# ljishen/bitar

Hardware: AMD Instinct MI355X
Metric: GiB/s compress+decompress on 1-GiB Arrow buffer, 1/2/4/8 GPUs; % HBM roofline (higher is better)
Workload: dtype u8; 1 GPU; LZ4 block compress + decompress round trip, 1 GiB per GPU, 64 KiB segments, Silesia-style mix (BASELINE configs[2]); bytes_per_gpu=1073741824, segment_bytes=65536, segments_per_gpu=16384, codec=lz4-block, input_kind=1, parallelism=1 GPU

## Files before the change

### bitar_amd/csrc/compress.hip

```cpp
#include "window_parse.hip.h"

namespace bitar_hip {

namespace cmp {

__device__ __forceinline__ uint32_t lane_sel(uint64_t m, uint32_t a, uint32_t b) {
  uint32_t r;
  __asm__("v_cndmask_b32_e64 %0, %1, %2, %3" : "=v"(r) : "v"(b), "v"(a), "s"(m));
  return r;
}

#ifndef BITAR_LZ4_GATHER
#define BITAR_LZ4_GATHER 2
#endif
#ifndef BITAR_LZ4_OBUF
#define BITAR_LZ4_OBUF 512
#endif
constexpr uint32_t kLz4Obuf = BITAR_LZ4_OBUF;
constexpr uint32_t kSeqCap = 64;
struct Lz4Lds {
#if BITAR_LZ4_GATHER == 2
  uint8_t ring[kLz4Obuf];
#else
  uint8_t ring[kLz4Obuf + kWave];
#endif
  uint2 seqs[kSeqCap + 1];
  uint32_t marks[kWave + 1];
};

struct Lz4Out : ByteOutT<kLz4Obuf> {
  Lz4Lds* L;
  uint32_t nseq;
  uint32_t last_end;
  uint32_t step_id;

  __device__ __forceinline__ void init(Lz4Lds* lds, GMEM uint8_t* d, uint64_t c) {
    L = lds;
    ring = lds->ring;
    dst = d;
    cap = c;
    op = flushed = 0;
    overflow = false;
    nseq = 0;
    last_end = 0;
    step_id = 0;
    lds->marks[lane_id()] = 0;
    lds_order();
  }
  __device__ __forceinline__ void put_ext(uint32_t v) {
    const uint32_t cnt = v / 255u + 1;
    for (uint32_t k = 0; k < cnt; k += kWave) {
      const uint32_t step = cnt - k < kWave ? cnt - k : kWave;
      if (!room(step)) return;
      const uint32_t t = k + lane_id();
      put(t + 1 < cnt ? 255u : v % 255u, step);
    }
  }
  __device__ __forceinline__ void one(const GMEM uint8_t* in, const InRing& I, uint32_t lit_start,
                                      uint32_t lit_len, uint32_t off, uint32_t mlen) {
    if (overflow) return;
    const uint32_t ml = mlen ? mlen - kMinMatch : 0;
    const uint32_t token = ((lit_len < 15 ? lit_len : 15) << 4) | (ml < 15 ? ml : 15);
    if (!room(1)) return;
    put(token, 1);
    if (lit_len >= 15) put_ext(lit_len - 15);
    if (overflow) return;
    if (lit_len) {
      if ((uint64_t)op + lit_len > cap) { overflow = true; return; }
      if (lit_len <= 256 && lit_start >= I.lo) {
        for (uint32_t k = 0; k < lit_len; k += kWave) {
          const uint32_t step = lit_len - k < kWave ? lit_len - k : kWave;
          room(step);
          lds_order();
          const uint32_t b = I.byte(lit_start + k + (lane_id() < step ? lane_id() : 0u));
          put(b, step);
        }
      } else {
        flush(op, true);
        wave_copy_global(dst + op, in + lit_start, lit_len);
        op += lit_len;
        flushed = op;
      }
    }
    if (!mlen) return;
    if (!room(2)) return;
    put(lane_id() ? off >> 8 : off & 0xFF, 2);
    if (ml >= 15) put_ext(ml - 15);
  }

#if BITAR_LZ4_GATHER == 2
  __device__ __forceinline__ bool bulk(const InRing& I, uint32_t lo, uint32_t hi, uint32_t q,
                                       uint32_t lit_start, uint32_t off, uint32_t mlen) {
    const uint32_t lane = lane_id();
    const bool in = (lane >= lo) & (lane < hi);
    const uint32_t lit_len = q - lit_start, ml = mlen - kMinMatch;
    const uint32_t nlx = lit_len >= 15 ? 1u : 0u, nmx = ml >= 15 ? 1u : 0u;
    const uint32_t e = in ? 3u + nlx + nmx + lit_len : 0u;
    const uint32_t incl = wave_incl_sum(e);
    const uint32_t total = readlane(incl, kWave - 1);
    if ((uint64_t)op + total > cap) return false;
    const uint32_t a = incl - e;
    const uint32_t tok = ((lit_len < 15 ? lit_len : 15) << 4) | (ml < 15 ? ml : 15);
    const uint32_t A = a + nlx;
    const uint32_t T1 = a + 2u + nlx + lit_len;
    const uint32_t hb = nlx ? tok | (((lit_len - 15u) & 0xFFu) << 8) : tok << 8;
    const uint32_t D = I.in_lo + lit_start - A - 2u;
    const uint32_t pA = A | (T1 << 16);
    const uint32_t pH = hb | (D << 16);
    const uint32_t pT = (off & 0xFFFFu) | (((ml - 15u) & 0xFFu) << 16);
    const uint32_t a4 = in ? a << 2 : 0x7FFFFF00u;
    const uint32_t mark = a + 1u;
    const uint32_t zero = 0;
    const uint32_t rbase = (uint32_t)(uintptr_t)dst + op - 1u;
    uint32_t u = lane + 1u;
    uint32_t before = lo - 1u;
    for (uint32_t R = 0; R < total; R += kWave) {
      if (op + kWave - flushed > kLz4Obuf - 64) flush(op, false);
      lds_order();
      const uint32_t slot = min(a4 - (R << 2), (uint32_t)kWave << 2);
      *reinterpret_cast<uint32_t*>(reinterpret_cast<uint8_t*>(L->marks) + slot) = mark;
      lds_order();
      const uint32_t mk = L->marks[lane];
      L->marks[lane] = zero;
      const uint64_t S = ballot(mk == u);
      const uint32_t base = before + (uint32_t)(S & 1u);
      const uint64_t S1 = S >> 1;
      const uint32_t idx = __builtin_amdgcn_mbcnt_hi((uint32_t)(S1 >> 32),
                                                     __builtin_amdgcn_mbcnt_lo((uint32_t)S1, 0u));
      before += (uint32_t)__builtin_popcountll(S);
      const int src = (int)((idx << 2) + (base << 2));
      const uint32_t qA = (uint32_t)__builtin_amdgcn_ds_bpermute(src, (int)pA);
      const uint32_t qH = (uint32_t)__builtin_amdgcn_ds_bpermute(src, (int)pH);
      const uint32_t qT = (uint32_t)__builtin_amdgcn_ds_bpermute(src, (int)pT);
      const uint32_t r = u - (qA & 0xFFFFu);
      const uint32_t t = u - (qA >> 16);
      const uint32_t sel = min(min(t, r + 4u), 6u);
      const uint32_t litb = I.ring[(((u << 16) + qH) >> 16) & I.mask];
      const uint32_t hi4 = __builtin_amdgcn_perm(litb, qH, 0x0C040100u);
      const uint32_t b = __builtin_amdgcn_perm(hi4, qT, sel);
      const uint32_t nb = total - R < kWave ? total - R : kWave;
      ring[(rbase + u) & kMask] = (uint8_t)b;
      lds_order();
      op += nb;
      u += kWave;
    }
    return true;
  }
#else
  __device__ __forceinline__ bool bulk(const InRing& I, uint32_t lo, uint32_t hi, uint32_t q,
                                       uint32_t lit_start, uint32_t off, uint32_t mlen) {
    const uint32_t lane = lane_id();
    const bool in = (lane >= lo) & (lane < hi);
    const uint32_t lit_len = q - lit_start, ml = mlen - kMinMatch;
    const uint32_t nlx = lit_len >= 15 ? 1u : 0u, nmx = ml >= 15 ? 1u : 0u;
    const uint32_t e = in ? 3u + nlx + nmx + lit_len : 0u;
    const uint32_t incl = wave_incl_sum(e);
    const uint32_t total = readlane(incl, kWave - 1);
    if ((uint64_t)op + total > cap) return false;
    const uint32_t a = incl - e;
    const uint32_t tok = ((lit_len < 15 ? lit_len : 15) << 4) | (ml < 15 ? ml : 15);
    const uint32_t p0 = a | (lit_len << 16) | (nlx << 25) | (nmx << 26);
    const uint32_t p1 = lit_start | (tok << 16);
    const uint32_t p2 = (off & 0xFFFFu) | (((ml - 15u) & 0xFFu) << 16) | ((lit_len - 15u) << 24);
    for (uint32_t R = 0; R < total; R += kWave) {
      room(kWave);
      step_id += 1;
      const bool st = in & (a - R < kWave);
      lds_order();
      L->marks[st ? a - R : kWave] = (step_id << 8) | (lane + 1);
      lds_order();
      const uint32_t mk = L->marks[lane];
      const uint32_t before = (uint32_t)__builtin_popcountll(ballot(in & (a < R)));
      const uint32_t carry = before ? lo + before : 0u;
      const uint32_t v = (mk >> 8) == step_id ? (mk & 0xFFu) : 0u;
      const uint32_t s1 = max(wave_incl_max(v), carry);
      const int src = (int)((s1 - 1) << 2);
      const uint32_t q0 = (uint32_t)__builtin_amdgcn_ds_bpermute(src, (int)p0);
      const uint32_t q1 = (uint32_t)__builtin_amdgcn_ds_bpermute(src, (int)p1);
      const uint32_t q2 = (uint32_t)__builtin_amdgcn_ds_bpermute(src, (int)p2);
      const uint32_t r = R + lane - (q0 & 0xFFFFu);
      const uint32_t ll = (q0 >> 16) & 511u;
      const uint32_t L0 = 1u + ((q0 >> 25) & 1u), h = L0 + ll;
      const uint32_t litb = I.byte((q1 & 0xFFFFu) + r - L0);
      uint32_t b = r == h + 2 ? (q2 >> 16) & 0xFFu : (q2 >> 8) & 0xFFu;
      b = r == h ? q2 & 0xFFu : b;
      b = r < h ? litb : b;
      b = r < L0 ? q2 >> 24 : b;
      b = r == 0 ? (q1 >> 16) & 0xFFu : b;
      const uint32_t nb = total - R < kWave ? total - R : kWave;
      lds_order();
      ring[lane < nb ? at(op + lane) : kLz4Obuf + lane] = (uint8_t)b;
      lds_order();
      op += nb;
    }
    return true;
  }
#endif

  __device__ __forceinline__ void flush_seqs(const GMEM uint8_t* in, const InRing& I) {
    const uint32_t cnt = nseq;
    nseq = 0;
    if (!cnt || overflow) return;
    const uint32_t lane = lane_id();
    lds_order();
    const uint2 rec = L->seqs[lane < cnt ? lane : kSeqCap];
    const uint32_t q = rec.x & 0xFFFFu, off = (rec.x >> 16) + 1u, mlen = rec.y;
    const uint32_t end = q + mlen;
    const uint32_t prev = wave_shr1(end);
    const uint32_t lit_start = lane == 0 ? last_end : prev;
    const uint32_t lit_len = q - lit_start;
    last_end = readlane(end, cnt - 1);
    const uint64_t live = cnt < kWave ? (1ull << cnt) - 1 : ~0ull;
    uint64_t special = (ballot(lit_len >= 270u) | ballot(mlen >= 270u + kMinMatch) |
                        ballot(lit_start < I.lo)) & live;
    uint32_t lo = 0;
    for (;;) {
      const uint32_t k = special ? (uint32_t)__builtin_ctzll(special) : cnt;
      if (k > lo && !bulk(I, lo, k, q, lit_start, off, mlen)) {
        for (uint32_t j = lo; j < k && !overflow; ++j)
          one(in, I, readlane(lit_start, j), readlane(lit_len, j), readlane(off, j),
              readlane(mlen, j));
      }
      if (k >= cnt || overflow) break;
      one(in, I, readlane(lit_start, k), readlane(lit_len, k), readlane(off, k),
          readlane(mlen, k));
      special &= special - 1;
      lo = k + 1;
    }
  }

  __device__ __forceinline__ void sequence(const GMEM uint8_t* in, const InRing& I,
                                           uint32_t lit_start, uint32_t lit_len, uint32_t off,
                                           uint32_t mlen) {
    flush_seqs(in, I);
    one(in, I, lit_start, lit_len, off, mlen);
  }
  __device__ __forceinline__ uint32_t pending_from(uint32_t anchor, uint32_t) const { return anchor; }

  __device__ __forceinline__ void between(const GMEM uint8_t* in, const InRing& I) {
    if (nseq > kSeqCap - 16) flush_seqs(in, I);
  }
  __device__ __forceinline__ void window(const GMEM uint8_t*, const InRing&, const Window& W,
                                         uint32_t, uint32_t) {
    if (!W.chain) return;
    const uint64_t chain = W.chain;
    const uint32_t idx = __builtin_amdgcn_mbcnt_hi((uint32_t)(chain >> 32),
                                                   __builtin_amdgcn_mbcnt_lo((uint32_t)chain, nseq));
    const uint32_t lane = lane_id();
    lds_order();
    L->seqs[lane_sel(chain, idx, kSeqCap)] =
        make_uint2((W.x + lane) | (W.dm1 << 16), W.mlen);
    lds_order();
    nseq += (uint32_t)__builtin_popcountll(chain);
  }
};

constexpr uint32_t kBitWords = BITAR_CMP_BITWORDS, kBitMask = kBitWords - 1;

__device__ __forceinline__ uint32_t rev(uint32_t v, uint32_t n) {
  return __builtin_bitreverse32(v) >> (32 - n);
}
__device__ __forceinline__ uint32_t fixed_code(uint32_t s, uint32_t& n) {
  const uint32_t code = s < 144 ? 0x30 + s : s < 256 ? 0x190 + (s - 144) : s < 280 ? s - 256 : 0xC0 + (s - 280);
  n = s < 144 ? 8u : s < 256 ? 9u : s < 280 ? 7u : 8u;
  return __builtin_bitreverse32(code) >> (32 - n);
}
__device__ __forceinline__ uint32_t match_code(uint32_t mlen, uint32_t off, uint32_t& n) {
  const uint32_t v = mlen - 3;
  const uint32_t lev = 29u - __builtin_clz(v | 8u);
  const uint32_t le = mlen == 258 || v < 8 ? 0u : lev;
  const uint32_t lc = mlen == 258 ? 28u : v < 8 ? v : 4 * lev + 4 + ((v >> lev) & 3u);
  const uint32_t lx = v & ((1u << le) - 1);
  const uint32_t d = off - 1;
  const uint32_t dev = 30u - __builtin_clz(d | 4u);
  const uint32_t de = d < 4 ? 0u : dev;
  const uint32_t dc = d < 4 ? d : 2 * dev + 2 + ((d >> dev) & 1u);
  const uint32_t dx = d & ((1u << de) - 1);
  uint32_t ln;
  const uint32_t code = fixed_code(257 + lc, ln);
  n = ln + le + 5 + de;
  return code | (lx << ln) | (rev(dc, 5) << (ln + le)) | (dx << (ln + le + 5));
}

#ifndef BITAR_DFL_BULK
#define BITAR_DFL_BULK 1
#endif
struct DflLds {
  uint2 recs[kSeqCap + 1];
  uint32_t marks[kWave + 1];
};
struct DflOut {
  uint32_t* stage;
  GMEM uint32_t* dst;
  uint64_t cap;
  uint64_t bits;
  uint32_t wflushed;
  bool overflow;

  __device__ __forceinline__ void flush_words(uint32_t upto) {
    const uint32_t lane = lane_id();
    lds_order();
    for (uint32_t w = wflushed + lane; w < upto; w += kWave) {
      dst[w] = stage[w & kBitMask];
      stage[w & kBitMask] = 0;
    }
    lds_order();
    wflushed = upto;
  }
  __device__ __forceinline__ void drain() {
    const uint32_t full = (uint32_t)(bits >> 5);
    if (full != wflushed) flush_words(full);
  }
  __device__ __forceinline__ void put_lanes(uint32_t val, uint32_t nb) {
    if (overflow) return;
    const uint32_t incl = wave_incl_sum(nb);
    const uint32_t total = readlane(incl, 63);
    if ((bits + total + 7) / 8 > cap) { overflow = true; return; }
    const uint64_t bp = bits + incl - nb;
    const uint32_t w = (uint32_t)(bp >> 5), sh = (uint32_t)(bp & 31);
    const uint32_t spill = sh + nb > 32 ? val >> ((32 - sh) & 31) : 0u;
    lds_order();
    if (nb) atomicOr(&stage[w & kBitMask], val << sh);
    if (sh + nb > 32) atomicOr(&stage[(w + 1) & kBitMask], spill);
    lds_order();
    bits += total;
    const uint32_t full = (uint32_t)(bits >> 5);
    if (full - wflushed >= kBitWords - 80) flush_words(full);
  }
  __device__ __forceinline__ void put_one(uint32_t val, uint32_t nb) {
    put_lanes(lane_id() == 0 ? val : 0u, lane_id() == 0 ? nb : 0u);
  }
  __device__ __forceinline__ void literals(const GMEM uint8_t* in, const InRing& I, uint32_t s,
                                           uint32_t n) {
    const uint32_t lane = lane_id();
    const bool ring_ok = s >= I.lo;
    for (uint32_t k = 0; k < n; k += kWave) {
      const uint32_t step = n - k < kWave ? n - k : kWave;
      const uint32_t q = s + k + (lane < step ? lane : 0);
      uint32_t b;
      lds_order();
      if (ring_ok) b = I.byte(q);
      else b = lane < step ? (uint32_t)in[q] : 0u;
      uint32_t nb;
      const uint32_t code = fixed_code(b, nb);
      put_lanes(lane < step ? code : 0u, lane < step ? nb : 0u);
      if (overflow) return;
    }
  }
#if BITAR_DFL_BULK
  DflLds* L;
  uint32_t npend, last_end;

  __device__ __forceinline__ void bulk(const InRing& I, uint32_t lo, uint32_t hi,
                                       uint32_t lit_start, uint32_t ll, uint32_t mv, uint32_t mb) {
    const uint32_t lane = lane_id();
    const bool in = (lane >= lo) & (lane < hi);
    const uint32_t e = in ? ll + 1u : 0u;
    const uint32_t incl = wave_incl_sum(e);
    const uint32_t total = readlane(incl, kWave - 1);
    const uint32_t a = incl - e;
    const uint32_t D = I.in_lo + lit_start - a - 1u;
    const uint32_t pX = ((a + ll + 1u) << 16) | mb;
    const uint32_t a4 = in ? a << 2 : 0x7FFFFF00u;
    const uint32_t mark = a + 1u;
    const uint32_t zero = 0;
    uint32_t u = lane + 1u;
    uint32_t before = lo - 1u;
    for (uint32_t R = 0; R < total && !overflow; R += kWave) {
      lds_order();
      const uint32_t slot = min(a4 - (R << 2), (uint32_t)kWave << 2);
      *reinterpret_cast<uint32_t*>(reinterpret_cast<uint8_t*>(L->marks) + slot) = mark;
      lds_order();
      const uint32_t mk = L->marks[lane];
      L->marks[lane] = zero;
      const uint64_t S = ballot(mk == u);
      const uint32_t base = before + (uint32_t)(S & 1u);
      const uint64_t S1 = S >> 1;
      const uint32_t k = __builtin_amdgcn_mbcnt_hi((uint32_t)(S1 >> 32),
                                                   __builtin_amdgcn_mbcnt_lo((uint32_t)S1, 0u));
      before += (uint32_t)__builtin_popcountll(S);
      const int src = (int)((k << 2) + (base << 2));
      const uint32_t qD = (uint32_t)__builtin_amdgcn_ds_bpermute(src, (int)D);
      const uint32_t qX = (uint32_t)__builtin_amdgcn_ds_bpermute(src, (int)pX);
      const uint32_t qM = (uint32_t)__builtin_amdgcn_ds_bpermute(src, (int)mv);
      const uint32_t b = I.ring[(qD + u) & I.mask];
      uint32_t lb;
      const uint32_t lv = fixed_code(b, lb);
      const bool ism = u == (qX >> 16);
      const bool live = u <= total;
      put_lanes(ism ? qM : lv, live ? (ism ? (qX & 63u) : lb) : 0u);
      u += kWave;
    }
  }
  __device__ __forceinline__ void flush_seqs(const GMEM uint8_t* in, const InRing& I) {
    const uint32_t cnt = npend;
    npend = 0;
    if (!cnt || overflow) return;
    const uint32_t lane = lane_id();
    lds_order();
    const uint2 rec = L->recs[lane < cnt ? lane : kSeqCap];
    const uint32_t q = rec.x & 0xFFFFu, off = (rec.x >> 16) + 1u, mlen = rec.y;
    const uint32_t end = q + mlen;
    const uint32_t prev = wave_shr1(end);
    const uint32_t lit_start = lane == 0 ? last_end : prev;
    const uint32_t ll = q - lit_start;
    last_end = readlane(end, cnt - 1);
    uint32_t mb;
    const uint32_t mv = match_code(lane < cnt ? mlen : 3u, lane < cnt ? off : 1u, mb);
    const uint64_t live = cnt < kWave ? (1ull << cnt) - 1 : ~0ull;
    uint64_t special = ballot(lit_start < I.lo) & ballot(ll != 0u) & live;
    uint32_t lo = 0;
    for (;;) {
      const uint32_t k = special ? (uint32_t)__builtin_ctzll(special) : cnt;
      if (k > lo) bulk(I, lo, k, lit_start, ll, mv, mb);
      if (k >= cnt || overflow) break;
      literals(in, I, readlane(lit_start, k), readlane(ll, k));
      put_one(readlane(mv, k), readlane(mb, k));
      special &= special - 1;
      lo = k + 1;
    }
  }
  __device__ __forceinline__ uint32_t pending_from(uint32_t anchor, uint32_t) const { return anchor; }
  __device__ __forceinline__ void between(const GMEM uint8_t* in, const InRing& I) {
    if (npend > kSeqCap - 16) flush_seqs(in, I);
  }
  __device__ __forceinline__ void sequence(const GMEM uint8_t* in, const InRing& I, uint32_t s,
                                           uint32_t n, uint32_t, uint32_t) {
    flush_seqs(in, I);
    literals(in, I, s, n);
  }
  __device__ __forceinline__ void window(const GMEM uint8_t*, const InRing&, const Window& W,
                                         uint32_t, uint32_t) {
    if (!W.chain) return;
    const uint64_t chain = W.chain;
    const uint32_t idx = __builtin_amdgcn_mbcnt_hi((uint32_t)(chain >> 32),
                                                   __builtin_amdgcn_mbcnt_lo((uint32_t)chain, npend));
    const uint32_t lane = lane_id();
    lds_order();
    L->recs[lane_sel(chain, idx, kSeqCap)] =
        make_uint2((W.x + lane) | (W.dm1 << 16), W.mlen);
    lds_order();
    npend += (uint32_t)__builtin_popcountll(chain);
  }
#else
  __device__ __forceinline__ uint32_t pending_from(uint32_t, uint32_t emitted) const { return emitted; }
  __device__ __forceinline__ void between(const GMEM uint8_t*, const InRing&) {}
  __device__ __forceinline__ void sequence(const GMEM uint8_t* in, const InRing& I, uint32_t s,
                                           uint32_t n, uint32_t, uint32_t) {
    literals(in, I, s, n);
  }

  __device__ __forceinline__ void window(const GMEM uint8_t*, const InRing&, const Window& W,
                                         uint32_t, uint32_t n) {
    const uint32_t lane = lane_id();
    const uint32_t q = W.x + lane;
    const bool cl = (W.chain >> lane) & 1;
    const uint32_t pend = wave_incl_max(cl ? q + W.mlen : 0u);
    const bool covered = q < W.pos_in || (!cl && q < pend);
    uint32_t mb, lb;
    const uint32_t mv = match_code(cl ? W.mlen : 3u, cl ? W.off() : 1u, mb);
    const uint32_t lv = fixed_code(W.byte, lb);
    const bool lit = !cl && !covered && q < n;
    put_lanes(cl ? mv : lit ? lv : 0u, cl ? mb : lit ? lb : 0u);
  }
#endif
};

}

#ifndef BITAR_LZ4C_WAVES
#define BITAR_LZ4C_WAVES 0
#endif
#if BITAR_LZ4C_WAVES
#define BITAR_LZ4C_ATTR __attribute__((amdgpu_waves_per_eu(BITAR_LZ4C_WAVES)))
#else
#define BITAR_LZ4C_ATTR
#endif
template <uint32_t RING, uint32_t HLOG>
__global__ __launch_bounds__(64) BITAR_LZ4C_ATTR void lz4_compress_kernel(
    const uint8_t* __restrict__ input, uint64_t n_total, uint32_t seg,
    uint8_t* __restrict__ slab, uint64_t slot_stride, uint8_t* const* __restrict__ dsts,
    uint32_t* __restrict__ sizes, uint32_t* __restrict__ err, const uint32_t* __restrict__ order) {
  using namespace cmp;
  __shared__ __attribute__((aligned(16))) uint16_t table[(1u << HLOG) + 8];
  __shared__ __attribute__((aligned(16))) uint8_t inring[RING + kInPad];
  __shared__ __attribute__((aligned(16))) Lz4Lds olds;
  const uint32_t i_seg = order ? order[blockIdx.x] : blockIdx.x;
  const uint64_t seg_off = (uint64_t)i_seg * seg;
  if (seg_off >= n_total) return;
  const uint32_t n = (uint32_t)((n_total - seg_off) < seg ? (n_total - seg_off) : seg);
  Lz4Out o;
  o.init(&olds, global_ptr(dsts ? dsts[i_seg] : slab + (uint64_t)i_seg * slot_stride), slot_stride);
#ifndef BITAR_CMP_LZ4_SKIP
#define BITAR_CMP_LZ4_SKIP 1
#endif
  parse<Lz4Out, false, BITAR_CMP_LZ4_SKIP != 0, RING, HLOG>(global_ptr(input + seg_off), n,
                                         global_ptr(input + n_total), table, inring,
                                         RING - 1536u, 0xFFFFFFFFu, o);
  o.flush(o.op, true);
  if (lane_id() == 0) {
    sizes[i_seg] = o.overflow ? 0xFFFFFFFFu : o.op;
    if (o.overflow) atomicOr(err, 2u);
  }
}

template __global__ void lz4_compress_kernel<cmp::kIn, cmp::kHashLog>(
    const uint8_t*, uint64_t, uint32_t, uint8_t*, uint64_t, uint8_t* const*, uint32_t*, uint32_t*,
    const uint32_t*);
template __global__ void lz4_compress_kernel<16384, 12>(
    const uint8_t*, uint64_t, uint32_t, uint8_t*, uint64_t, uint8_t* const*, uint32_t*, uint32_t*,
    const uint32_t*);

template <bool BITS>
__device__ __forceinline__ void deflate_compress_body(
    const uint8_t* __restrict__ input, uint64_t n_total, uint32_t seg,
    uint8_t* __restrict__ slab, uint64_t slot_stride, uint8_t* const* __restrict__ dsts,
    uint32_t* __restrict__ sizes, uint32_t* __restrict__ err, const uint32_t* __restrict__ order,
    uint32_t* __restrict__ bits) {
  using namespace cmp;
  __shared__ __attribute__((aligned(16))) uint16_t table[1u << kHashLog];
  __shared__ __attribute__((aligned(16))) uint8_t inring[kIn + kInPad];
  __shared__ __attribute__((aligned(16))) uint32_t stage[kBitWords];
#if BITAR_DFL_BULK
  __shared__ __attribute__((aligned(16))) DflLds dl;
#endif
  const uint32_t i_seg = order ? order[blockIdx.x] : blockIdx.x;
  const uint64_t seg_off = (uint64_t)i_seg * seg;
  if (seg_off >= n_total) return;
  const uint32_t n = (uint32_t)((n_total - seg_off) < seg ? (n_total - seg_off) : seg);
  for (uint32_t k = lane_id(); k < kBitWords; k += kWave) stage[k] = 0;
  DflOut o;
  o.stage = stage;
  o.dst = reinterpret_cast<GMEM uint32_t*>(
      global_ptr(dsts ? dsts[i_seg] : slab + (uint64_t)i_seg * slot_stride));
  o.cap = slot_stride;
  o.bits = 0;
  o.wflushed = 0;
  o.overflow = false;
#if BITAR_DFL_BULK
  o.L = &dl;
  o.npend = 0;
  o.last_end = 0;
  dl.marks[lane_id()] = 0;
  lds_order();
#endif
  o.put_one(1u | (1u << 1), 3);
  parse(global_ptr(input + seg_off), n, global_ptr(input + n_total), table, inring, kMaxDist,
        258u, o);
  uint32_t eb;
  const uint32_t eob = fixed_code(256, eb);
  o.put_one(eob, eb);
  o.flush_words((uint32_t)((o.bits + 31) >> 5));
  uint32_t size = (uint32_t)((o.bits + 7) >> 3);
  uint32_t nbits = (uint32_t)o.bits;
  const uint32_t nblk = (n + 65534u) / 65535u;
  const uint32_t stored = nblk * 5u + n;
  if (!o.overflow && stored < size + (n >> 4)) {
    GMEM uint8_t* d = reinterpret_cast<GMEM uint8_t*>(o.dst);
    const GMEM uint8_t* in = global_ptr(input + seg_off);
    global_fence_wave();
    uint32_t p = 0, q = 0;
    for (uint32_t b = 0; b < nblk; ++b) {
      const uint32_t len = n - p < 65535u ? n - p : 65535u;
      const uint32_t lane = lane_id();
      const uint32_t hv = lane == 0 ? (b + 1 == nblk ? 1u : 0u)
                          : lane == 1 ? len & 0xFFu : lane == 2 ? len >> 8
                          : lane == 3 ? ~len & 0xFFu : (~len >> 8) & 0xFFu;
      if (lane < 5) d[q + lane] = (uint8_t)hv;
      wave_copy_global(d + q + 5, in + p, len);
      p += len;
      q += 5 + len;
    }
    size = stored;
    nbits = stored * 8u;
  }
  if (lane_id() == 0) {
    sizes[i_seg] = o.overflow ? 0xFFFFFFFFu : size;
    if (BITS && bits) bits[i_seg] = o.overflow ? 0xFFFFFFFFu : nbits;
    if (o.overflow) atomicOr(err, 2u);
  }
}

__global__ __launch_bounds__(64) void deflate_compress_kernel(
    const uint8_t* __restrict__ input, uint64_t n_total, uint32_t seg,
    uint8_t* __restrict__ slab, uint64_t slot_stride, uint8_t* const* __restrict__ dsts,
    uint32_t* __restrict__ sizes, uint32_t* __restrict__ err, const uint32_t* __restrict__ order) {
  deflate_compress_body<false>(input, n_total, seg, slab, slot_stride, dsts, sizes, err, order,
                               nullptr);
}

__global__ __launch_bounds__(64) void deflate_compress_bits_kernel(
    const uint8_t* __restrict__ input, uint64_t n_total, uint32_t seg,
    uint8_t* __restrict__ slab, uint64_t slot_stride, uint8_t* const* __restrict__ dsts,
    uint32_t* __restrict__ sizes, uint32_t* __restrict__ err, const uint32_t* __restrict__ order,
    uint32_t* __restrict__ bits) {
  deflate_compress_body<true>(input, n_total, seg, slab, slot_stride, dsts, sizes, err, order,
                              bits);
}

}
```

Before: 244.1 GiB/s.

## Add ring-direct LZ4 sequence emitter with mark-based literal gather

Adds a third bulk emitter and makes it the default. Each lane writes its token, extension bytes and offset straight into the LDS output ring, using masked selects that send inactive lanes to a trash slot. Literal bytes are gathered a wave-width at a time: owner lanes are found by marking LDS slots and balloting, and their source and destination bases are fetched with ds_permute/bpermute. This replaces the previous packed prefix-sum gather and chunks the work so the ring is flushed before it overflows. The cost is extra LDS traffic and barriers for every 64-byte literal chunk.

```diff
diff --git a/bitar_amd/csrc/compress.hip b/bitar_amd/csrc/compress.hip
--- a/bitar_amd/csrc/compress.hip
+++ b/bitar_amd/csrc/compress.hip
@@ -11,7 +11,7 @@
 }
 
 #ifndef BITAR_LZ4_GATHER
-#define BITAR_LZ4_GATHER 2
+#define BITAR_LZ4_GATHER 3
 #endif
 #ifndef BITAR_LZ4_OBUF
 #define BITAR_LZ4_OBUF 512
@@ -19,7 +19,9 @@
 constexpr uint32_t kLz4Obuf = BITAR_LZ4_OBUF;
 constexpr uint32_t kSeqCap = 64;
 struct Lz4Lds {
-#if BITAR_LZ4_GATHER == 2
+#if BITAR_LZ4_GATHER == 3
+  uint8_t ring[kLz4Obuf + 16];
+#elif BITAR_LZ4_GATHER == 2
   uint8_t ring[kLz4Obuf];
 #else
   uint8_t ring[kLz4Obuf + kWave];
@@ -88,7 +90,86 @@
     if (ml >= 15) put_ext(ml - 15);
   }
 
-#if BITAR_LZ4_GATHER == 2
+#if BITAR_LZ4_GATHER == 3
+  __device__ __forceinline__ bool bulk(const InRing& I, uint32_t lo, uint32_t hi, uint32_t q,
+                                       uint32_t lit_start, uint32_t off, uint32_t mlen) {
+    constexpr uint32_t kTrash = kLz4Obuf, kLim = kLz4Obuf - 64;
+    const uint32_t lane = lane_id();
+    const bool in = (lane >= lo) & (lane < hi);
+    const uint32_t lit_len = q - lit_start, ml = mlen - kMinMatch;
+    const uint32_t nlx = lit_len >= 15 ? 1u : 0u, nmx = ml >= 15 ? 1u : 0u;
+    const uint32_t e = in ? (3u + nlx + nmx + lit_len) | (lit_len << 16) : 0u;
+    const uint32_t incl = wave_incl_sum(e);
+    const uint32_t total = readlane(incl, kWave - 1) & 0xFFFFu;
+    if ((uint64_t)op + total > cap) return false;
+    const uint32_t excl = incl - e;
+    const uint32_t a = excl & 0xFFFFu, lp = excl >> 16;
+    const uint32_t iend = incl & 0xFFFFu;
+    const uint32_t tok = ((lit_len < 15 ? lit_len : 15) << 4) | (ml < 15 ? ml : 15);
+    const uint32_t tA = (uint32_t)(uintptr_t)dst + op + a;
+    const uint32_t tO = tA + 1u + nlx + lit_len;
+    const uint32_t x0 = tA & kMask, x1 = (tA + 1u) & kMask;
+    const uint32_t x2 = tO & kMask, x3 = (tO + 1u) & kMask, x4 = (tO + 2u) & kMask;
+    const uint64_t lxm = ballot(nlx != 0u), mxm = ballot(nmx != 0u);
+    const bool ne = in & (lit_len != 0u);
+    const uint64_t nem = ballot(ne);
+    const uint32_t rank = __builtin_amdgcn_mbcnt_hi((uint32_t)(nem >> 32),
+                                                    __builtin_amdgcn_mbcnt_lo((uint32_t)nem, 0u));
+    const uint32_t Din = I.in_lo + lit_start - lp - 1u;
+    const uint32_t Dout = tA + nlx - lp;
+    const uint32_t Pc = (uint32_t)__builtin_amdgcn_ds_permute(
+        (int)((ne ? rank : kWave - 1) << 2), (int)((Din & 0xFFFFu) | (Dout << 16)));
+    const uint32_t lp4 = ne ? lp << 2 : 0x7FFFFF00u;
+    const uint32_t mark = lp + 1u;
+    const uint32_t zero = 0;
+    uint32_t u = lane + 1u;
+    uint32_t before = 0;
+    uint32_t c0 = lo, ba = 0, bl = 0;
+    do {
+      const uint64_t over = ballot(iend > ba + kLim);
+      uint32_t c1 = over ? (uint32_t)__builtin_ctzll(over) : kWave;
+      c1 = c1 < hi ? c1 : hi;
+      c1 = c1 > c0 ? c1 : c0 + 1u;
+      const uint32_t end = readlane(incl, c1 - 1);
+      const uint32_t ea = end & 0xFFFFu, el = end >> 16;
+      if (op + (ea - ba) - flushed > kLim) flush(op, false);
+      lds_order();
+      const uint64_t cm = ((c1 < kWave ? 1ull << c1 : 0ull) - 1ull) & ~((1ull << c0) - 1ull);
+      ring[lane_sel(cm, x0, kTrash)] = (uint8_t)tok;
+      ring[lane_sel(cm & lxm, x1, kTrash)] = (uint8_t)(lit_len - 15u);
+      ring[lane_sel(cm, x2, kTrash)] = (uint8_t)off;
+      ring[lane_sel(cm, x3, kTrash)] = (uint8_t)(off >> 8);
+      ring[lane_sel(cm & mxm, x4, kTrash)] = (uint8_t)(ml - 15u);
+      for (uint32_t R = bl; R < el; R += kWave) {
+        const uint32_t nb = el - R < kWave ? el - R : kWave;
+        const uint64_t vm = nb < kWave ? (1ull << nb) - 1ull : ~0ull;
+        lds_order();
+        const uint32_t slot = min(lp4 - (R << 2), (uint32_t)kWave << 2);
+        *reinterpret_cast<uint32_t*>(reinterpret_cast<uint8_t*>(L->marks) + slot) = mark;
+        lds_order();
+        const uint32_t mk = L->marks[lane];
+        L->marks[lane] = zero;
+        const uint64_t S = ballot(mk == u) & vm;
+        const uint32_t base = before - 1u + (uint32_t)(S & 1u);
+        const uint64_t S1 = S >> 1;
+        const uint32_t k = __builtin_amdgcn_mbcnt_hi((uint32_t)(S1 >> 32),
+                                                     __builtin_amdgcn_mbcnt_lo((uint32_t)S1, 0u));
+        before += (uint32_t)__builtin_popcountll(S);
+        const uint32_t p = (uint32_t)__builtin_amdgcn_ds_bpermute((int)((k << 2) + (base << 2)),
+                                                                  (int)Pc);
+        const uint32_t b = I.ring[(p + u) & I.mask];
+        ring[lane_sel(vm, ((p >> 16) + u) & kMask, kTrash)] = (uint8_t)b;
+        u += nb;
+      }
+      lds_order();
+      op += ea - ba;
+      ba = ea;
+      bl = el;
+      c0 = c1;
+    } while (c0 < hi);
+    return true;
+  }
+#elif BITAR_LZ4_GATHER == 2
   __device__ __forceinline__ bool bulk(const InRing& I, uint32_t lo, uint32_t hi, uint32_t q,
                                        uint32_t lit_start, uint32_t off, uint32_t mlen) {
     const uint32_t lane = lane_id();
```

Measured after the change: 250.5 GiB/s, median of 6. +2.6%, better.
